# Eden-Kramer-Lab/spectral_connectivity

Measured on AMD Instinct MI355X. Metric: channel-pair*freq-bins/s for CSM+coherence(+wPLI), higher is better.
Workload: dtype f32

## Files before the change

spectral_connectivity_amd/csrc/sc_fused2.hip:

```cpp
#include <stdlib.h>
#include "sc_fused_common.h"

typedef _Float16 h16x4 __attribute__((ext_vector_type(4)));
typedef _Float16 h16x8 __attribute__((ext_vector_type(8)));
typedef _Float16 h16x2 __attribute__((ext_vector_type(2)));
typedef __attribute__((address_space(3))) unsigned char lds_u8;
typedef short s16x4 __attribute__((ext_vector_type(4)));
typedef __attribute__((address_space(3))) s16x4 lds_s16x4;

#define F2_GROUP 1056
#define F2_PLANE (8 * F2_GROUP + 64)
#define F2_NPL 6
#define F2_HPL 4
#define F2_BUF (F2_NPL * F2_PLANE)
#define F2_NBUF 3
#define F2_SCALE_OFF (F2_NBUF * F2_BUF)
#define F2_LDS (F2_SCALE_OFF + 512)
#define F2_ROW_TILE 256

extern "C" int64_t sc_planes_scales_work_bytes(int64_t n_rows, int64_t width);
extern "C" int64_t sc_planes_row_bytes(int64_t n_signals) { return (int64_t)F2_ROW_TILE * ((n_signals + 31) / 32); }

__device__ __forceinline__ unsigned f2_pack(float lo, float hi) {
    const h16x2 v = {(_Float16)lo, (_Float16)hi};
    return __builtin_bit_cast(unsigned, v);
}
__device__ __forceinline__ float f2_lo(unsigned p) { return (float)__builtin_bit_cast(h16x2, p)[0]; }
__device__ __forceinline__ float f2_hi(unsigned p) { return (float)__builtin_bit_cast(h16x2, p)[1]; }
__device__ __forceinline__ void f2_split2(float x0, float x1, unsigned& h, unsigned& m) {
    h = f2_pack(x0, x1);
    m = f2_pack(x0 - f2_lo(h), x1 - f2_hi(h));
}

__device__ __forceinline__ float planes_mag(float v) {
    const float a = fabsf(v);
    return a <= 3.4028234e38f ? a : 0.f;
}
__device__ __forceinline__ float planes_fin(float v) { return fabsf(v) <= 3.4028234e38f ? v : 0.f; }
__global__ void __launch_bounds__(256) planes_absmax_kernel(const float* x, int64_t n_rows, int width, int comps, unsigned* mx, float* part) {
    __shared__ unsigned red[2048];
    __shared__ float sred[2048];
    const int64_t rows_per_block = (n_rows + gridDim.x - 1) / gridDim.x;
    const int64_t r0 = (int64_t)blockIdx.x * rows_per_block, r1 = r0 + rows_per_block < n_rows ? r0 + rows_per_block : n_rows;
    const int tid = threadIdx.x;
    auto ord = [](float v) -> unsigned { const unsigned u = __float_as_uint(v); return (u & 0x80000000u) ? ~u : (u | 0x80000000u); };
    if ((width & 3) == 0 && width <= 1024 && (((uintptr_t)x) & 15) == 0 && r0 < r1) {
        const int q = width >> 2;
        const int rows_per_step = 256 / q;
        const int cq = tid % q, ro = tid / q;
        for (int i = tid; i < 2 * width; i += 256) red[i] = 0u;
        __syncthreads();
        if (ro < rows_per_step) {
            float4 pv = make_float4(0.f, 0.f, 0.f, 0.f);
            if (part) {
                pv = *reinterpret_cast<const float4*>(x + r0 * width + 4 * cq);
                pv.x = planes_fin(pv.x); pv.y = planes_fin(pv.y); pv.z = planes_fin(pv.z); pv.w = planes_fin(pv.w);
            }
            float4 hi = make_float4(-3.4e38f, -3.4e38f, -3.4e38f, -3.4e38f), lo = hi;
            float4 m = make_float4(0.f, 0.f, 0.f, 0.f), s1 = m, s2 = m;
            auto take = [&](const float4 v) {
                if (part) {
                    const float a0 = planes_fin(v.x), a1 = planes_fin(v.y), a2 = planes_fin(v.z), a3 = planes_fin(v.w);
                    const bool f0 = fabsf(v.x) <= 3.4028234e38f, f1 = fabsf(v.y) <= 3.4028234e38f, f2 = fabsf(v.z) <= 3.4028234e38f,
                               f3 = fabsf(v.w) <= 3.4028234e38f;
                    hi.x = fmaxf(hi.x, f0 ? a0 : hi.x); hi.y = fmaxf(hi.y, f1 ? a1 : hi.y); hi.z = fmaxf(hi.z, f2 ? a2 : hi.z); hi.w = fmaxf(hi.w, f3 ? a3 : hi.w);
                    lo.x = fmaxf(lo.x, f0 ? -a0 : lo.x); lo.y = fmaxf(lo.y, f1 ? -a1 : lo.y); lo.z = fmaxf(lo.z, f2 ? -a2 : lo.z); lo.w = fmaxf(lo.w, f3 ? -a3 : lo.w);
                    const float d0 = f0 ? a0 - pv.x : 0.f, d1 = f1 ? a1 - pv.y : 0.f, d2 = f2 ? a2 - pv.z : 0.f, d3 = f3 ? a3 - pv.w : 0.f;
                    s1.x += d0; s1.y += d1; s1.z += d2; s1.w += d3;
                    s2.x = fmaf(d0, d0, s2.x); s2.y = fmaf(d1, d1, s2.y); s2.z = fmaf(d2, d2, s2.z); s2.w = fmaf(d3, d3, s2.w);
                } else {
                    m.x = fmaxf(m.x, planes_mag(v.x)); m.y = fmaxf(m.y, planes_mag(v.y));
                    m.z = fmaxf(m.z, planes_mag(v.z)); m.w = fmaxf(m.w, planes_mag(v.w));
                }
            };
            int64_t r = r0 + ro;
            for (; r + 3 * rows_per_step < r1; r += 4 * rows_per_step) {
                float4 v[4];
#pragma unroll
                for (int u = 0; u < 4; ++u) v[u] = *reinterpret_cast<const float4*>(x + (r + (int64_t)u * rows_per_step) * width + 4 * cq);
#pragma unroll
                for (int u = 0; u < 4; ++u) take(v[u]);
            }
            for (; r < r1; r += rows_per_step) take(*reinterpret_cast<const float4*>(x + r * width + 4 * cq));
            if (part) {
                atomicMax(red + 4 * cq, ord(hi.x)); atomicMax(red + 4 * cq + 1, ord(hi.y)); atomicMax(red + 4 * cq + 2, ord(hi.z)); atomicMax(red + 4 * cq + 3, ord(hi.w));
                atomicMax(red + width + 4 * cq, ord(lo.x)); atomicMax(red + width + 4 * cq + 1, ord(lo.y));
                atomicMax(red + width + 4 * cq + 2, ord(lo.z)); atomicMax(red + width + 4 * cq + 3, ord(lo.w));
                float* sr = sred + (ro * width + 4 * cq) * 2;
                sr[0] = s1.x; sr[1] = s2.x; sr[2] = s1.y; sr[3] = s2.y; sr[4] = s1.z; sr[5] = s2.z; sr[6] = s1.w; sr[7] = s2.w;
            } else {
                atomicMax(red + 4 * cq, __float_as_uint(m.x)); atomicMax(red + 4 * cq + 1, __float_as_uint(m.y));
                atomicMax(red + 4 * cq + 2, __float_as_uint(m.z)); atomicMax(red + 4 * cq + 3, __float_as_uint(m.w));
            }
        }
        __syncthreads();
        for (int col = tid; col < width; col += 256) {
            if (!part) {
                if (red[col]) atomicMax(mx + col / comps, red[col]);
                continue;
            }
            if (red[col]) atomicMax(mx + col, red[col]);
            if (red[width + col]) atomicMax(mx + width + col, red[width + col]);
            float t1 = 0.f, t2 = 0.f;
            for (int k = 0; k < rows_per_step; ++k) { t1 += sred[(k * width + col) * 2]; t2 += sred[(k * width + col) * 2 + 1]; }
            float* o = part + ((int64_t)blockIdx.x * width + col) * 3;
            o[0] = planes_fin(x[r0 * width + col]); o[1] = t1; o[2] = t2;
        }
        return;
    }
    for (int col = tid; col < width; col += 256) {
        float m = 0.f, hi = -3.4e38f, lo = -3.4e38f, t1 = 0.f, t2 = 0.f;
        const float pv = (part && r0 < r1) ? planes_fin(x[r0 * width + col]) : 0.f;
        bool any = false;
        for (int64_t r = r0; r < r1; ++r) {
            const float v = x[r * width + col];
            m = fmaxf(m, planes_mag(v));
            if (fabsf(v) <= 3.4028234e38f) { any = true; hi = fmaxf(hi, v); lo = fmaxf(lo, -v); const float d = v - pv; t1 += d; t2 = fmaf(d, d, t2); }
        }
        if (!part) { if (m > 0.f) atomicMax(mx + col / comps, __float_as_uint(m)); continue; }
        if (any) { atomicMax(mx + col, ord(hi)); atomicMax(mx + width + col, ord(lo)); }
        float* o = part + ((int64_t)blockIdx.x * width + col) * 3;
        o[0] = pv; o[1] = t1; o[2] = t2;
    }
}
__global__ void planes_scale_kernel(const unsigned* mx, int C, float factor, float* scale) {
    const int c = blockIdx.x * blockDim.x + threadIdx.x;
    if (c >= C) return;
    const float b = __uint_as_float(mx[c]) * factor;
    float s = 1.f;
    if (b > 0.f && b < 3.0e38f) {
        int e;
        (void)frexpf(b, &e);
        int k = 15 - e;
        k = k < -100 ? -100 : (k > 100 ? 100 : k);
        s = ldexpf(1.f, k);
    }
    scale[c] = s;
    scale[C + c] = 1.f / s;
}
__global__ void __launch_bounds__(64) planes_scale_quality_kernel(unsigned* mx, int C, float taper_abs_sum, int detrend, float* scale,
                                                                  const float* part, int n_blocks, int64_t rows_per_block, int64_t n_rows) {
    const int c = blockIdx.x, lane = threadIdx.x;
    auto unord = [](unsigned p) -> float { return __uint_as_float((p & 0x80000000u) ? (p & 0x7fffffffu) : ~p); };
    const unsigned ph = mx[c], pl = mx[C + c];
    const bool any = ph != 0u && pl != 0u;
    const float hi = any ? unord(ph) : 0.f, lo = any ? -unord(pl) : 0.f;
    const float amp = detrend ? 4.f * (hi - lo) : fmaxf(fabsf(hi), fabsf(lo));
    const float b = amp * taper_abs_sum;
    float s = 1.f;
    if (b > 0.f && b < 3.0e38f) {
        int e;
        (void)frexpf(b, &e);
        int k = 15 - e;
        k = k < -100 ? -100 : (k > 100 ? 100 : k);
        s = ldexpf(1.f, k);
    }
    if (lane == 0) { scale[c] = s; scale[C + c] = 1.f / s; }
    float quiet = 3.4e38f;
    for (int blk = lane; blk < n_blocks; blk += 64) {
        const int64_t rb = (int64_t)blk * rows_per_block;
        const double nb = (double)((rb + rows_per_block < n_rows ? rb + rows_per_block : n_rows) - rb);
        if (nb < 2.0) continue;
        const float* o = part + ((int64_t)blk * C + c) * 3;
        const double s1 = (double)o[1], s2 = (double)o[2];
        const double var = (s2 - s1 * s1 / nb) / nb, mean = (double)o[0] + s1 / nb;
        if (!(var > 1e-12 * (mean * mean + 1e-300))) continue;
        const float typ = (float)sqrt(detrend ? var : var + mean * mean);
        quiet = fminf(quiet, typ);
    }
    for (int off = 32; off >= 1; off >>= 1) quiet = fminf(quiet, __shfl_down(quiet, off, 64));
    if (lane == 0 && quiet < 3.0e38f && b > 0.f && b < 3.0e38f) atomicMin(mx + 2 * C, __float_as_uint(quiet * s));
}
static int64_t planes_stat_blocks(int64_t n_rows) {
    int64_t blocks = n_rows / 128;
    return blocks < 1 ? 1 : (blocks > 2048 ? 2048 : blocks);
}
extern "C" int64_t sc_planes_scales_work_bytes(int64_t n_rows, int64_t width) {
    return 4 * ((2 * width + 1 + 3) / 4 * 4) + 4 * 3 * planes_stat_blocks(n_rows) * width;
}
static int planes_scales(const float* d_x, int64_t n_rows, int C, int comps, float factor, float* d_scale, void* d_work, void* stream) {
    hipStream_t s = (hipStream_t)stream;
    unsigned* mx = (unsigned*)d_work;
    SC_CHECK_HIP(hipMemsetAsync(mx, 0, sizeof(unsigned) * C, s));
    hipLaunchKernelGGL(planes_absmax_kernel, dim3((unsigned)planes_stat_blocks(n_rows)), dim3(256), 0, s, d_x, n_rows, C * comps, comps, mx, (float*)nullptr);
    hipLaunchKernelGGL(planes_scale_kernel, dim3((C + 63) / 64), dim3(64), 0, s, mx, C, factor, d_scale);
    SC_CHECK_HIP(hipGetLastError());
    return SC_OK;
}
extern "C" int sc_planes_scales_from_series_f32(const float* d_x, int64_t T, int64_t R, int64_t C, double taper_abs_sum,
                                                float* d_scale, void* d_work, void* stream) {
    ScTimed timed_("planes_scales", stream);
    SC_REQUIRE(d_x && d_scale && d_work && T >= 1 && R >= 1 && C >= 1 && taper_abs_sum > 0.0, "bad argument");
    return planes_scales(d_x, T * R, (int)C, 1, (float)(8.0 * taper_abs_sum), d_scale, d_work, stream);
}
extern "C" int sc_planes_scales_quality_f32(const float* d_x, int64_t T, int64_t R, int64_t C, int detrend_type, double taper_abs_sum,
                                            float* d_scale, void* d_work, int64_t work_bytes, float* d_quality, void* stream) {
    ScTimed timed_("planes_scales", stream);
    SC_REQUIRE(d_x && d_scale && d_work && d_quality && T >= 1 && R >= 1 && C >= 1 && taper_abs_sum > 0.0, "bad argument");
    SC_REQUIRE(detrend_type >= 0 && detrend_type <= 2, "unknown detrend_type");
    SC_REQUIRE(work_bytes >= sc_planes_scales_work_bytes(T * R, C), "work buffer smaller than sc_planes_scales_work_bytes");
    hipStream_t s = (hipStream_t)stream;
    unsigned* mx = (unsigned*)d_work;
    const int64_t n_rows = T * R, blocks = planes_stat_blocks(n_rows), head = (2 * C + 1 + 3) / 4 * 4;
    float* part = (float*)d_work + head;
    SC_CHECK_HIP(hipMemsetAsync(mx, 0, sizeof(unsigned) * 2 * C, s));
    SC_CHECK_HIP(hipMemsetAsync(mx + 2 * C, 0x7f, sizeof(unsigned), s));
    hipLaunchKernelGGL(planes_absmax_kernel, dim3((unsigned)blocks), dim3(256), 0, s, d_x, n_rows, (int)C, 1, mx, part);
    hipLaunchKernelGGL(planes_scale_quality_kernel, dim3((unsigned)C), dim3(64), 0, s, mx, (int)C, (float)taper_abs_sum,
                       detrend_type != SC_DETREND_NONE ? 1 : 0, d_scale, part, (int)blocks, (n_rows + blocks - 1) / blocks, n_rows);
    SC_CHECK_HIP(hipMemcpyAsync(d_quality, mx + 2 * C, sizeof(float), hipMemcpyDeviceToDevice, s));
    SC_CHECK_HIP(hipGetLastError());
    return SC_OK;
}
extern "C" int sc_planes_scales_from_spectra_f32(const void* d_X, int64_t n_rows, int64_t C, float* d_scale, void* d_work, void* stream) {
    SC_REQUIRE(d_X && d_scale && d_work && n_rows >= 1 && C >= 1, "bad argument");
    return planes_scales((const float*)d_X, n_rows, (int)C, 2, 1.0f, d_scale, d_work, stream);
}

struct PlanesConvArgs {
    const float2* X;
    unsigned char* P;
    const float* scale;
    int64_t sF, sW, sR, sK;
    int F, W, R, K, C, nct;
    int64_t n_rows;
};
__global__ void __launch_bounds__(256) planes_from_spectra_kernel(PlanesConvArgs a) {
    const int pairs_per_row = a.nct * 16;
    const int64_t i = (int64_t)blockIdx.x * 256 + threadIdx.x;
    if (i >= a.n_rows * pairs_per_row) return;
    const int64_t row = i / pairs_per_row;
    const int pr = (int)(i - row * pairs_per_row), c = 2 * pr;
    int64_t t = row;
    const int k = (int)(t % a.K); t /= a.K;
    const int r = (int)(t % a.R); t /= a.R;
    const int w = (int)(t % a.W); t /= a.W;
    const int f = (int)t;
    const float2* src = a.X + (int64_t)f * a.sF + (int64_t)w * a.sW + (int64_t)r * a.sR + (int64_t)k * a.sK + c;
    float2 v0 = make_float2(0.f, 0.f), v1 = v0;
    if (c < a.C) { const float s0 = a.scale[c]; v0 = src[0]; v0.x *= s0; v0.y *= s0; }
    if (c + 1 < a.C) { const float s1 = a.scale[c + 1]; v1 = src[1]; v1.x *= s1; v1.y *= s1; }
    unsigned* dst = reinterpret_cast<unsigned*>(a.P + row * (int64_t)a.nct * F2_ROW_TILE + (pr >> 4) * F2_ROW_TILE) + (pr & 15);
    unsigned rh, rm, ih, im;
    f2_split2(v0.x, v1.x, rh, rm);
    f2_split2(v0.y, v1.y, ih, im);
    dst[0] = rh; dst[16] = rm; dst[32] = ih; dst[48] = im;
}
__global__ void __launch_bounds__(256) spectra_from_planes_kernel(PlanesConvArgs a) {
    const int pairs_per_row = a.nct * 16;
    const int64_t i = (int64_t)blockIdx.x * 256 + threadIdx.x;
    if (i >= a.n_rows * pairs_per_row) return;
    const int64_t row = i / pairs_per_row;
    const int pr = (int)(i - row * pairs_per_row), c = 2 * pr;
    if (c >= a.C) return;
    int64_t t = row;
    const int k = (int)(t % a.K); t /= a.K;
    const int r = (int)(t % a.R); t /= a.R;
    const int w = (int)(t % a.W); t /= a.W;
    const int f = (int)t;
    const unsigned* src = reinterpret_cast<const unsigned*>(a.P + row * (int64_t)a.nct * F2_ROW_TILE + (pr >> 4) * F2_ROW_TILE) + (pr & 15);
    const unsigned rh = src[0], rm = src[16], ih = src[32], im = src[48];
    const float i0 = a.scale[a.C + c], i1 = (c + 1 < a.C) ? a.scale[a.C + c + 1] : 1.f;
    const float2 v0 = make_float2((f2_lo(rh) + f2_lo(rm)) * i0, (f2_lo(ih) + f2_lo(im)) * i0);
    const float2 v1 = make_float2((f2_hi(rh) + f2_hi(rm)) * i1, (f2_hi(ih) + f2_hi(im)) * i1);
    float2* dst = const_cast<float2*>(a.X) + (int64_t)f * a.sF + (int64_t)w * a.sW + (int64_t)r * a.sR + (int64_t)k * a.sK + c;
    dst[0] = v0;
    if (c + 1 < a.C) dst[1] = v1;
}
static int planes_conv(const void* d_X, const sc_spectra_desc* d, const float* d_scale, void* d_P, bool to_planes, void* stream) {
    SC_REQUIRE(d_X && d && d_P && d_scale, "NULL argument");
    SC_REQUIRE(d->n_freq >= 1 && d->n_windows >= 1 && d->n_trials >= 1 && d->n_tapers >= 1 && d->n_signals >= 1, "empty dimension");
    PlanesConvArgs a;
    a.X = (const float2*)d_X; a.P = (unsigned char*)d_P; a.scale = d_scale;
    a.sF = d->stride_freq; a.sW = d->stride_window; a.sR = d->stride_trial; a.sK = d->stride_taper;
    a.F = (int)d->n_freq; a.W = (int)d->n_windows; a.R = (int)d->n_trials; a.K = (int)d->n_tapers; a.C = (int)d->n_signals;
    a.nct = (a.C + 31) / 32;
    a.n_rows = (int64_t)a.F * a.W * a.R * a.K;
    const int64_t items = a.n_rows * a.nct * 16;
    const unsigned blocks = (unsigned)((items + 255) / 256);
    if (to_planes) hipLaunchKernelGGL(planes_from_spectra_kernel, dim3(blocks), dim3(256), 0, (hipStream_t)stream, a);
    else hipLaunchKernelGGL(spectra_from_planes_kernel, dim3(blocks), dim3(256), 0, (hipStream_t)stream, a);
    SC_CHECK_HIP(hipGetLastError());
    return SC_OK;
}
extern "C" int sc_planes_from_spectra_f32(const void* d_X, const sc_spectra_desc* desc, const float* d_scale, void* d_P, void* stream) {
    ScTimed timed_("planes_from_spectra", stream);
    return planes_conv(d_X, desc, d_scale, d_P, true, stream);
}
extern "C" int sc_spectra_from_planes_f32(const void* d_P, const sc_spectra_desc* desc, const float* d_scale, void* d_X, void* stream) {
    ScTimed timed_("spectra_from_planes", stream);
    return planes_conv(d_X, desc, d_scale, const_cast<void*>(d_P), false, stream);
}

struct Fused2Args {
    FusedArgs f;
    const unsigned char* P;
    const float* inv_scale;
    int64_t row_bytes;
    int64_t obs_rows;
    int loader_csm;
    int terms4;
    int fold_obs;
};

__device__ __forceinline__ h16x4 f2_tr(lds_u8* base, int off) {
    return __builtin_bit_cast(h16x4, __builtin_amdgcn_ds_read_tr16_b64_v4i16((lds_s16x4*)(base + off)));
}
__device__ __forceinline__ h16x8 f2_frag(lds_u8* base, int p) {
    const h16x4 a = f2_tr(base, p * F2_PLANE), b = f2_tr(base, p * F2_PLANE + 256);
    const h16x8 v = {a[0], a[1], a[2], a[3], b[0], b[1], b[2], b[3]};
    return v;
}

#define F2_MFMA(a, b, c) c = __builtin_amdgcn_mfma_f32_16x16x32_f16(a, b, c, 0, 0, 0)

struct F2Loader {
    const unsigned char* src;
    unsigned voff;
    int lds_off;
    int o7_0, plane;
    int n_inst;
};
template <int NHALF>
__device__ __forceinline__ F2Loader f2_loader(const Fused2Args& a, int wave, const unsigned char* part_base) {
    F2Loader L;
    const int lane = fu_lane();
    const int piece = lane & 15, ct = NHALF == 2 ? ((piece >> 2) & 1) : (piece >> 2), half = NHALF == 2 ? (piece >> 3) : 0;
    if (a.loader_csm) {
        L.plane = wave < 4 ? wave : -1;
        L.o7_0 = 0;
        L.n_inst = 8;
    } else {
        L.plane = wave >= 4 ? ((wave - 4) & 3) : -1;
        L.o7_0 = wave >= 4 ? 4 * ((wave - 4) >> 2) : 0;
        L.n_inst = 4;
    }
    L.voff = (unsigned)((8 * (lane >> 4) + FU_OC * half) * a.obs_rows * a.row_bytes + fu_byte(a.f.map.off32, ct) * F2_ROW_TILE + (piece & 3) * 16);
    L.src = part_base + (L.plane < 0 ? 0 : L.plane) * 64;
    L.lds_off = (L.plane < 0 ? 0 : L.plane) * F2_PLANE + L.o7_0 * F2_GROUP;
    return L;
}
template <int NHALF>
__device__ __forceinline__ void f2_issue(const Fused2Args& a, const F2Loader& L, lds_u8* buf, int o0, int n_left) {
    if (L.plane < 0) return;
    const int lane = fu_lane();
    const int ct = NHALF == 2 ? ((lane >> 2) & 1) : ((lane & 15) >> 2);
    const bool lane_ok = ct < a.f.NB32 && fu_byte(a.f.map.n32, ct) > 0;
    const int o_first = L.o7_0 + 8 * (lane >> 4) + (NHALF == 2 ? FU_OC * ((lane >> 3) & 1) : 0);
#pragma unroll
    for (int i = 0; i < 8; ++i) {
        if (i >= L.n_inst) break;
        lds_u8* dst = buf + L.lds_off + i * F2_GROUP;
        const unsigned char* src = L.src + (int64_t)(o0 + L.o7_0 + i) * a.obs_rows * a.row_bytes;
        if (lane_ok && o_first + i < n_left)
            asm volatile("s_mov_b32 m0, %0\n\ts_nop 0\n\tglobal_load_lds_dwordx4 %1, %2"
                         :: "s"((unsigned)reinterpret_cast<uintptr_t>(dst)), "v"(L.voff), "s"(src) : "memory", "m0");
    }
}
template <int NHALF>
__device__ __forceinline__ void f2_finish(const F2Loader& L, lds_u8* buf, int n_left) {
    if (L.plane < 0) return;
    const int lane = fu_lane();
    if (n_left < FU_OC * NHALF) {
#pragma unroll
        for (int i = 0; i < 8; ++i) {
            if (i >= L.n_inst) break;
            const int o = L.o7_0 + i + 8 * (lane >> 4) + (NHALF == 2 ? FU_OC * ((lane >> 3) & 1) : 0);
            if (o >= n_left)
                *reinterpret_cast<__attribute__((address_space(3))) u32x4*>(buf + L.lds_off + i * F2_GROUP + 16 * lane) = (u32x4){0u, 0u, 0u, 0u};
        }
    }
    if (L.plane < 2) {
#pragma unroll
        for (int i = 0; i < 8; ++i) {
            if (i >= L.n_inst) break;
            lds_u8* g = buf + L.lds_off + i * F2_GROUP + 16 * lane;
            u32x4 v = *reinterpret_cast<__attribute__((address_space(3))) u32x4*>(g);
            v[0] ^= 0x80008000u; v[1] ^= 0x80008000u; v[2] ^= 0x80008000u; v[3] ^= 0x80008000u;
            *reinterpret_cast<__attribute__((address_space(3))) u32x4*>(g + 4 * F2_PLANE) = v;
        }
    }
}

__device__ __forceinline__ int f2_issued(const F2Loader& L, int n_left) {
    if (L.plane < 0) return 0;
    const int k = n_left - L.o7_0;
    return k < 0 ? 0 : (k > L.n_inst ? L.n_inst : k);
}
__device__ __forceinline__ void f2_wait_loads(int outstanding) {
    switch (outstanding) {
    case 8: asm volatile("s_waitcnt vmcnt(8)" ::: "memory"); break;
    case 7: asm volatile("s_waitcnt vmcnt(7)" ::: "memory"); break;
    case 6: asm volatile("s_waitcnt vmcnt(6)" ::: "memory"); break;
    case 5: asm volatile("s_waitcnt vmcnt(5)" ::: "memory"); break;
    case 4: asm volatile("s_waitcnt vmcnt(4)" ::: "memory"); break;
    case 3: asm volatile("s_waitcnt vmcnt(3)" ::: "memory"); break;
    case 2: asm volatile("s_waitcnt vmcnt(2)" ::: "memory"); break;
    case 1: asm volatile("s_waitcnt vmcnt(1)" ::: "memory"); break;
    default: asm volatile("s_waitcnt vmcnt(0)" ::: "memory"); break;
    }
}

template <int NB32>
__device__ __forceinline__ void f2_mfma_role(const Fused2Args& a, lds_u8* lds, const unsigned char* lds_generic, const F2Loader& L,
                                             int wave, float* rec, int n_part) {
    const FusedArgs& p = a.f;
    constexpr int MAXS = 2 * NB32 + 1;
    constexpr int NHALF = NB32 <= 2 ? 2 : 1, CH = FU_OC * NHALF;
    const int FLUSH = a.fold_obs / CH;
    const unsigned sg = (unsigned)__builtin_amdgcn_readfirstlane((int)(wave == 0 ? p.seg0 : (wave == 1 ? p.seg1 : (wave == 2 ? p.seg2 : p.seg3))));
    const unsigned sg_n = (unsigned)__builtin_amdgcn_readfirstlane((int)((p.seg_n >> (8 * wave)) & 0xffu));
    const int rA_ = sg & 0xf, cA_ = (sg >> 4) & 0xf, rB_ = (sg >> 8) & 0xf, cB_ = (sg >> 12) & 0xf;
    const int nA_ = sg_n & 0xf, nB_ = sg_n >> 4;
    const int total = nA_ + nB_;
    f32x4 re[MAXS], im[MAXS];
#pragma unroll
    for (int s = 0; s < MAXS; ++s) { re[s] = (f32x4){0.f, 0.f, 0.f, 0.f}; im[s] = re[s]; }
    const int n_chunks = (n_part + CH - 1) / CH;
    float* out = rec + (int64_t)p.csm_plane * p.n_tiles * SC_TILE_ELEMS;
    const bool do_csm = p.csm_plane >= 0 && (p.debug_skip & 1) == 0;
    const bool loads = !(p.debug_skip & 8);
    const bool t4 = a.terms4 != 0;
    for (int ch = 0; ch < n_chunks; ++ch) {
        lds_u8* cur = lds + (loads ? (ch % F2_NBUF) : 0) * F2_BUF;
        const bool more = ch + 1 < n_chunks && loads, more2 = ch + 2 < n_chunks && loads;
        if (more2) f2_issue<NHALF>(a, L, lds + ((ch + 2) % F2_NBUF) * F2_BUF, (ch + 2) * CH, n_part - (ch + 2) * CH);
        if (do_csm && total > 0) {
            int rA = rA_, rB = rB_, nA = nA_, cA = cA_, cB = cB_;
            asm volatile("" : "+s"(rA), "+s"(rB), "+s"(nA), "+s"(cA), "+s"(cB));
            const int lane = fu_lane(), g = lane >> 4;
            lds_u8* b00 = cur + ((4 * (g & 1) + ((lane >> 2) & 3)) * F2_GROUP + 2 * (g >> 1) * 256 + (lane & 3) * 8);
            h16x8 arh, arm, aih, aim, nrh, nrm;
#pragma unroll
            for (int hv = 0; hv < NHALF; ++hv) {
            lds_u8* b0 = b00 + hv * 128;
#pragma unroll
            for (int s = 0; s < MAXS; ++s) {
                if (s < total) {
                    const bool in_a = s < nA;
                    const int row = in_a ? rA : rB;
                    const int col = in_a ? cA + s : cB + (s - nA);
                    if (s == 0 || s == nA) {
                        lds_u8* fa = b0 + row * 32;
                        arh = f2_frag(fa, 0); arm = f2_frag(fa, 1); aih = f2_frag(fa, 2); aim = f2_frag(fa, 3);
                        nrh = f2_frag(fa, 4); nrm = f2_frag(fa, 5);
                    }
                    lds_u8* fb = b0 + col * 32;
                    const h16x8 brh = f2_frag(fb, 0), bih = f2_frag(fb, 2), brm = f2_frag(fb, 1), bim = f2_frag(fb, 3);
                    F2_MFMA(arh, brh, re[s]);  F2_MFMA(aih, brh, im[s]);
                    F2_MFMA(aih, bih, re[s]);  F2_MFMA(nrh, bih, im[s]);
                    F2_MFMA(arh, brm, re[s]);  F2_MFMA(aih, brm, im[s]);
                    F2_MFMA(aih, bim, re[s]);  F2_MFMA(nrh, bim, im[s]);
                    F2_MFMA(arm, brh, re[s]);  F2_MFMA(aim, brh, im[s]);
                    F2_MFMA(aim, bih, re[s]);  F2_MFMA(nrm, bih, im[s]);
                    if (t4) {
                        F2_MFMA(arm, brm, re[s]);  F2_MFMA(aim, brm, im[s]);
                        F2_MFMA(aim, bim, re[s]);  F2_MFMA(nrm, bim, im[s]);
                    }
                }
            }
            }
        }
        if (more && L.plane >= 0) {
            f2_wait_loads(more2 ? f2_issued(L, n_part - (ch + 2) * CH) : 0);
            f2_finish<NHALF>(L, lds + ((ch + 1) % F2_NBUF) * F2_BUF, n_part - (ch + 1) * CH);
        }
        {
            const bool last = ch + 1 == n_chunks;
#pragma unroll
            for (int s = 0; s < MAXS; ++s) {
                const int f_s = FLUSH - 1 - s;
                const bool due = ((ch + 1 + s) % FLUSH) == 0 && !(p.debug_skip & 64);
                if (s < total && (due || last) && p.csm_plane >= 0) {
                    const bool first = ch <= f_s || (p.debug_skip & 64);
                    const bool in_a = s < nA_;
                    const int row = in_a ? rA_ : rB_;
                    const int col = in_a ? cA_ + s : cB_ + (s - nA_);
                    float* o_re = out + (int64_t)sc_tile_index(fu_gt(p.map, row), fu_gt(p.map, col), p.map.NBr) * SC_TILE_ELEMS;
                    float* o_im = o_re + (int64_t)p.n_tiles * SC_TILE_ELEMS;
                    const unsigned fl = (unsigned)fu_lane();
                    const unsigned base_idx = (fl >> 4) * 64u + (fl & 15u);
                    const float* isc = reinterpret_cast<const float*>((const unsigned char*)lds_generic + F2_SCALE_OFF);
                    const float sj = isc[col * 16 + (int)(fl & 15u)];
                    const f32x4 si = *reinterpret_cast<const f32x4*>(isc + row * 16 + 4 * (int)(fl >> 4));
#pragma unroll
                    for (int r = 0; r < 4; ++r) {
                        const unsigned idx = base_idx + 16u * r;
                        const float sc = sj * si[r];
                        if (first) {
                            o_re[idx] = re[s][r] * sc;
                            o_im[idx] = im[s][r] * sc;
                        } else {
                            unsafeAtomicAdd(o_re + idx, re[s][r] * sc);
                            unsafeAtomicAdd(o_im + idx, im[s][r] * sc);
                        }
                    }
                    re[s] = (f32x4){0.f, 0.f, 0.f, 0.f}; im[s] = re[s];
                }
            }
        }
        F2_BARRIER();
    }
    const int wps = 8 / p.n_sets;
    for (int half = wps >> 1; half >= 1; half >>= 1) { __syncthreads(); __syncthreads(); }
}

template <int NB32, int COL_LO, int ROW_HI, int SET, int OP, int RPW>
__device__ __forceinline__ void f2_valu_body(const Fused2Args& a, lds_u8* lds, unsigned char* smem, const F2Loader& L, int tid,
                                             int rsub, int wps, float* rec, int n_part) {
    const FusedArgs& p = a.f;
    using Tab = FuTab<NB32, COL_LO, ROW_HI, SET>;
    constexpr int NBLK = Tab::NBLK;
    constexpr bool PK = NBLK <= 4 && fu_nsets(NB32, COL_LO, ROW_HI) == 1;
// ... 307 lines not shown
```

Baseline: 2.788 billion.

## Split quality scan into dedicated kernel with per-slab records, drop memsets and global atomics

Adds a dedicated planes_scan_kernel that writes per-slab records (pivot, sums, hi/lo ordered max) in a column-major layout. The merge kernel then reduces those records per channel with a wave shuffle instead of using global atomicMax. The scan is software-pipelined with a 6-deep register prefetch and sched barriers. The separate memsets and the device-to-device copy of the quality value are removed, since the quality word is initialized inside the scan kernel and written directly. The aim is to cut launch and API overhead and atomic traffic in the scale/quality stage, at the cost of a larger work buffer and more per-channel merge reads.

```diff
diff --git a/spectral_connectivity_amd/csrc/sc_fused2.hip b/spectral_connectivity_amd/csrc/sc_fused2.hip
--- a/spectral_connectivity_amd/csrc/sc_fused2.hip
+++ b/spectral_connectivity_amd/csrc/sc_fused2.hip
@@ -37,41 +37,26 @@
     return a <= 3.4028234e38f ? a : 0.f;
 }
 __device__ __forceinline__ float planes_fin(float v) { return fabsf(v) <= 3.4028234e38f ? v : 0.f; }
-__global__ void __launch_bounds__(256) planes_absmax_kernel(const float* x, int64_t n_rows, int width, int comps, unsigned* mx, float* part) {
-    __shared__ unsigned red[2048];
-    __shared__ float sred[2048];
+static int64_t planes_stat_blocks(int64_t n_rows) {
+    int64_t blocks = n_rows / 128;
+    return blocks < 1 ? 1 : (blocks > 2048 ? 2048 : blocks);
+}
+__global__ void __launch_bounds__(256) planes_absmax_kernel(const float* x, int64_t n_rows, int width, int comps, unsigned* mx) {
+    __shared__ unsigned red[1024];
     const int64_t rows_per_block = (n_rows + gridDim.x - 1) / gridDim.x;
     const int64_t r0 = (int64_t)blockIdx.x * rows_per_block, r1 = r0 + rows_per_block < n_rows ? r0 + rows_per_block : n_rows;
     const int tid = threadIdx.x;
-    auto ord = [](float v) -> unsigned { const unsigned u = __float_as_uint(v); return (u & 0x80000000u) ? ~u : (u | 0x80000000u); };
     if ((width & 3) == 0 && width <= 1024 && (((uintptr_t)x) & 15) == 0 && r0 < r1) {
         const int q = width >> 2;
         const int rows_per_step = 256 / q;
         const int cq = tid % q, ro = tid / q;
-        for (int i = tid; i < 2 * width; i += 256) red[i] = 0u;
+        for (int i = tid; i < width; i += 256) red[i] = 0u;
         __syncthreads();
         if (ro < rows_per_step) {
-            float4 pv = make_float4(0.f, 0.f, 0.f, 0.f);
-            if (part) {
-                pv = *reinterpret_cast<const float4*>(x + r0 * width + 4 * cq);
-                pv.x = planes_fin(pv.x); pv.y = planes_fin(pv.y); pv.z = planes_fin(pv.z); pv.w = planes_fin(pv.w);
-            }
-            float4 hi = make_float4(-3.4e38f, -3.4e38f, -3.4e38f, -3.4e38f), lo = hi;
-            float4 m = make_float4(0.f, 0.f, 0.f, 0.f), s1 = m, s2 = m;
+            float4 m = make_float4(0.f, 0.f, 0.f, 0.f);
             auto take = [&](const float4 v) {
-                if (part) {
-                    const float a0 = planes_fin(v.x), a1 = planes_fin(v.y), a2 = planes_fin(v.z), a3 = planes_fin(v.w);
-                    const bool f0 = fabsf(v.x) <= 3.4028234e38f, f1 = fabsf(v.y) <= 3.4028234e38f, f2 = fabsf(v.z) <= 3.4028234e38f,
-                               f3 = fabsf(v.w) <= 3.4028234e38f;
-                    hi.x = fmaxf(hi.x, f0 ? a0 : hi.x); hi.y = fmaxf(hi.y, f1 ? a1 : hi.y); hi.z = fmaxf(hi.z, f2 ? a2 : hi.z); hi.w = fmaxf(hi.w, f3 ? a3 : hi.w);
-                    lo.x = fmaxf(lo.x, f0 ? -a0 : lo.x); lo.y = fmaxf(lo.y, f1 ? -a1 : lo.y); lo.z = fmaxf(lo.z, f2 ? -a2 : lo.z); lo.w = fmaxf(lo.w, f3 ? -a3 : lo.w);
-                    const float d0 = f0 ? a0 - pv.x : 0.f, d1 = f1 ? a1 - pv.y : 0.f, d2 = f2 ? a2 - pv.z : 0.f, d3 = f3 ? a3 - pv.w : 0.f;
-                    s1.x += d0; s1.y += d1; s1.z += d2; s1.w += d3;
-                    s2.x = fmaf(d0, d0, s2.x); s2.y = fmaf(d1, d1, s2.y); s2.z = fmaf(d2, d2, s2.z); s2.w = fmaf(d3, d3, s2.w);
-                } else {
-                    m.x = fmaxf(m.x, planes_mag(v.x)); m.y = fmaxf(m.y, planes_mag(v.y));
-                    m.z = fmaxf(m.z, planes_mag(v.z)); m.w = fmaxf(m.w, planes_mag(v.w));
-                }
+                m.x = fmaxf(m.x, planes_mag(v.x)); m.y = fmaxf(m.y, planes_mag(v.y));
+                m.z = fmaxf(m.z, planes_mag(v.z)); m.w = fmaxf(m.w, planes_mag(v.w));
             };
             int64_t r = r0 + ro;
             for (; r + 3 * rows_per_step < r1; r += 4 * rows_per_step) {
@@ -82,45 +67,18 @@
                 for (int u = 0; u < 4; ++u) take(v[u]);
             }
             for (; r < r1; r += rows_per_step) take(*reinterpret_cast<const float4*>(x + r * width + 4 * cq));
-            if (part) {
-                atomicMax(red + 4 * cq, ord(hi.x)); atomicMax(red + 4 * cq + 1, ord(hi.y)); atomicMax(red + 4 * cq + 2, ord(hi.z)); atomicMax(red + 4 * cq + 3, ord(hi.w));
-                atomicMax(red + width + 4 * cq, ord(lo.x)); atomicMax(red + width + 4 * cq + 1, ord(lo.y));
-                atomicMax(red + width + 4 * cq + 2, ord(lo.z)); atomicMax(red + width + 4 * cq + 3, ord(lo.w));
-                float* sr = sred + (ro * width + 4 * cq) * 2;
-                sr[0] = s1.x; sr[1] = s2.x; sr[2] = s1.y; sr[3] = s2.y; sr[4] = s1.z; sr[5] = s2.z; sr[6] = s1.w; sr[7] = s2.w;
-            } else {
-                atomicMax(red + 4 * cq, __float_as_uint(m.x)); atomicMax(red + 4 * cq + 1, __float_as_uint(m.y));
-                atomicMax(red + 4 * cq + 2, __float_as_uint(m.z)); atomicMax(red + 4 * cq + 3, __float_as_uint(m.w));
-            }
+            atomicMax(red + 4 * cq, __float_as_uint(m.x)); atomicMax(red + 4 * cq + 1, __float_as_uint(m.y));
+            atomicMax(red + 4 * cq + 2, __float_as_uint(m.z)); atomicMax(red + 4 * cq + 3, __float_as_uint(m.w));
         }
         __syncthreads();
-        for (int col = tid; col < width; col += 256) {
-            if (!part) {
-                if (red[col]) atomicMax(mx + col / comps, red[col]);
-                continue;
-            }
-            if (red[col]) atomicMax(mx + col, red[col]);
-            if (red[width + col]) atomicMax(mx + width + col, red[width + col]);
-            float t1 = 0.f, t2 = 0.f;
-            for (int k = 0; k < rows_per_step; ++k) { t1 += sred[(k * width + col) * 2]; t2 += sred[(k * width + col) * 2 + 1]; }
-            float* o = part + ((int64_t)blockIdx.x * width + col) * 3;
-            o[0] = planes_fin(x[r0 * width + col]); o[1] = t1; o[2] = t2;
-        }
+        for (int col = tid; col < width; col += 256)
+            if (red[col]) atomicMax(mx + col / comps, red[col]);
         return;
     }
     for (int col = tid; col < width; col += 256) {
-        float m = 0.f, hi = -3.4e38f, lo = -3.4e38f, t1 = 0.f, t2 = 0.f;
-        const float pv = (part && r0 < r1) ? planes_fin(x[r0 * width + col]) : 0.f;
-        bool any = false;
-        for (int64_t r = r0; r < r1; ++r) {
-            const float v = x[r * width + col];
-            m = fmaxf(m, planes_mag(v));
-            if (fabsf(v) <= 3.4028234e38f) { any = true; hi = fmaxf(hi, v); lo = fmaxf(lo, -v); const float d = v - pv; t1 += d; t2 = fmaf(d, d, t2); }
-        }
-        if (!part) { if (m > 0.f) atomicMax(mx + col / comps, __float_as_uint(m)); continue; }
-        if (any) { atomicMax(mx + col, ord(hi)); atomicMax(mx + width + col, ord(lo)); }
-        float* o = part + ((int64_t)blockIdx.x * width + col) * 3;
-        o[0] = pv; o[1] = t1; o[2] = t2;
+        float m = 0.f;
+        for (int64_t r = r0; r < r1; ++r) m = fmaxf(m, planes_mag(x[r * width + col]));
+        if (m > 0.f) atomicMax(mx + col / comps, __float_as_uint(m));
     }
 }
 __global__ void planes_scale_kernel(const unsigned* mx, int C, float factor, float* scale) {
@@ -138,11 +96,137 @@
     scale[c] = s;
     scale[C + c] = 1.f / s;
 }
-__global__ void __launch_bounds__(64) planes_scale_quality_kernel(unsigned* mx, int C, float taper_abs_sum, int detrend, float* scale,
-                                                                  const float* part, int n_blocks, int64_t rows_per_block, int64_t n_rows) {
+#define PLANES_SCAN_ROWS 6
+#define PLANES_NO_CHANNEL 0x7f7f7f7fu
+__global__ void __launch_bounds__(256, 8) planes_scan_kernel(const float* x, int64_t n_rows, int width, unsigned* rec, unsigned* quality) {
+    __shared__ uint4 sred[1024];
+    const int n_blocks = gridDim.x, slab = blockIdx.x;
+    const int64_t rows_per_block = (n_rows + n_blocks - 1) / n_blocks;
+    const int64_t r0 = (int64_t)slab * rows_per_block, r1 = r0 + rows_per_block < n_rows ? r0 + rows_per_block : n_rows;
+    const int tid = threadIdx.x;
+    if (blockIdx.x == 0 && tid == 0) *quality = PLANES_NO_CHANNEL;
+    auto ord = [](float v) -> unsigned { const unsigned u = __float_as_uint(v); return (u & 0x80000000u) ? ~u : (u | 0x80000000u); };
+    auto put = [&](int col, float pivot, float t1, float t2, unsigned hi, unsigned lo) {
+        unsigned* o = rec + ((int64_t)col * n_blocks + slab) * 5;
+        o[0] = __float_as_uint(pivot); o[1] = __float_as_uint(t1); o[2] = __float_as_uint(t2); o[3] = hi; o[4] = lo;
+    };
+    if ((width & 3) == 0 && width <= 1024 && (((uintptr_t)x) & 15) == 0 && r0 < r1) {
+        const int q = width >> 2;
+        const int rows_per_step = 256 / q;
+        const int cq = tid % q, ro = tid / q;
+        const float* xb = x + r0 * width;
+        const float p0 = tid < width ? xb[tid] : 0.f;
+        if (ro < rows_per_step) {
+            float4 pv = *reinterpret_cast<const float4*>(xb + 4 * cq);
+            pv.x = planes_fin(pv.x); pv.y = planes_fin(pv.y); pv.z = planes_fin(pv.z); pv.w = planes_fin(pv.w);
+            float4 hi = make_float4(-3.4e38f, -3.4e38f, -3.4e38f, -3.4e38f), lo = hi;
+            float4 s1 = make_float4(0.f, 0.f, 0.f, 0.f), s2 = s1;
+            auto take = [&](const float4 v) {
+                const float a0 = planes_fin(v.x), a1 = planes_fin(v.y), a2 = planes_fin(v.z), a3 = planes_fin(v.w);
+                const bool f0 = fabsf(v.x) <= 3.4028234e38f, f1 = fabsf(v.y) <= 3.4028234e38f, f2 = fabsf(v.z) <= 3.4028234e38f,
+                           f3 = fabsf(v.w) <= 3.4028234e38f;
+                hi.x = fmaxf(hi.x, f0 ? a0 : hi.x); hi.y = fmaxf(hi.y, f1 ? a1 : hi.y); hi.z = fmaxf(hi.z, f2 ? a2 : hi.z); hi.w = fmaxf(hi.w, f3 ? a3 : hi.w);
+                lo.x = fmaxf(lo.x, f0 ? -a0 : lo.x); lo.y = fmaxf(lo.y, f1 ? -a1 : lo.y); lo.z = fmaxf(lo.z, f2 ? -a2 : lo.z); lo.w = fmaxf(lo.w, f3 ? -a3 : lo.w);
+                const float d0 = f0 ? a0 - pv.x : 0.f, d1 = f1 ? a1 - pv.y : 0.f, d2 = f2 ? a2 - pv.z : 0.f, d3 = f3 ? a3 - pv.w : 0.f;
+                s1.x += d0; s1.y += d1; s1.z += d2; s1.w += d3;
+                s2.x = fmaf(d0, d0, s2.x); s2.y = fmaf(d1, d1, s2.y); s2.z = fmaf(d2, d2, s2.z); s2.w = fmaf(d3, d3, s2.w);
+            };
+            const int slab_rows = (int)(r1 - r0), step = rows_per_step * width;
+            const int mine = (slab_rows - ro + rows_per_step - 1) / rows_per_step;
+            const int full = slab_rows / rows_per_step / PLANES_SCAN_ROWS * PLANES_SCAN_ROWS;
+            const unsigned toff = (unsigned)(ro * width + 4 * cq);
+            const float* xs = xb;
+            float4 v[PLANES_SCAN_ROWS];
+            auto load = [&](int u) { v[u] = *reinterpret_cast<const float4*>(xs + u * step + toff); };
+            auto load_end = [&](int u) { v[u] = *reinterpret_cast<const float4*>(full + u < mine ? xs + u * step + toff : xb + 4 * cq); };
+            if (full > 0) {
+#pragma unroll
+                for (int u = 0; u < PLANES_SCAN_ROWS; ++u) load(u);
+                for (int k = PLANES_SCAN_ROWS; k < full; k += PLANES_SCAN_ROWS) {
+                    xs += (int64_t)PLANES_SCAN_ROWS * step;
+#pragma unroll
+                    for (int u = 0; u < PLANES_SCAN_ROWS; ++u) { take(v[u]); load(u); __builtin_amdgcn_sched_barrier(0); }
+                }
+                xs += (int64_t)PLANES_SCAN_ROWS * step;
+#pragma unroll
+                for (int u = 0; u < PLANES_SCAN_ROWS; ++u) { take(v[u]); load_end(u); __builtin_amdgcn_sched_barrier(0); }
+            } else {
+#pragma unroll
+                for (int u = 0; u < PLANES_SCAN_ROWS; ++u) load_end(u);
+            }
+#pragma unroll
+            for (int u = 0; u < PLANES_SCAN_ROWS; ++u)
+                if (full + u < mine) take(v[u]);
+            uint4* sr = sred + ro * width + 4 * cq;
+            sr[0] = make_uint4(__float_as_uint(s1.x), __float_as_uint(s2.x), ord(hi.x), ord(lo.x));
+            sr[1] = make_uint4(__float_as_uint(s1.y), __float_as_uint(s2.y), ord(hi.y), ord(lo.y));
+            sr[2] = make_uint4(__float_as_uint(s1.z), __float_as_uint(s2.z), ord(hi.z), ord(lo.z));
+            sr[3] = make_uint4(__float_as_uint(s1.w), __float_as_uint(s2.w), ord(hi.w), ord(lo.w));
+        }
+        __syncthreads();
+#pragma unroll
+        for (int j = 0; j < 4; ++j) {
+            const int col = tid + 256 * j;
+            if (col >= width) break;
+            float t1 = 0.f, t2 = 0.f;
+            unsigned ph = 0u, pl = 0u;
+            for (int k = 0; k < rows_per_step; ++k) {
+                const uint4 e = sred[k * width + col];
+                t1 += __uint_as_float(e.x); t2 += __uint_as_float(e.y);
+                ph = e.z > ph ? e.z : ph; pl = e.w > pl ? e.w : pl;
+            }
+            put(col, planes_fin(j == 0 ? p0 : xb[col]), t1, t2, ph, pl);
+        }
+        return;
+    }
+    for (int col = tid; col < width; col += 256) {
+        float hi = -3.4e38f, lo = -3.4e38f, t1 = 0.f, t2 = 0.f;
+        const float pv = r0 < r1 ? planes_fin(x[r0 * width + col]) : 0.f;
+        bool any = false;
+        for (int64_t r = r0; r < r1; ++r) {
+            const float v = x[r * width + col];
+            if (fabsf(v) <= 3.4028234e38f) { any = true; hi = fmaxf(hi, v); lo = fmaxf(lo, -v); const float d = v - pv; t1 += d; t2 = fmaf(d, d, t2); }
+        }
+        put(col, pv, t1, t2, any ? ord(hi) : 0u, any ? ord(lo) : 0u);
+    }
+}
+#define PLANES_MERGE_RECS 4
+__global__ void __launch_bounds__(64) planes_scale_quality_kernel(const unsigned* rec, int C, float taper_abs_sum, int detrend, float* scale,
+                                                                  unsigned* quality, int n_blocks, int64_t rows_per_block, int64_t n_rows) {
     const int c = blockIdx.x, lane = threadIdx.x;
+    const unsigned* rc = rec + (int64_t)c * n_blocks * 5;
     auto unord = [](unsigned p) -> float { return __uint_as_float((p & 0x80000000u) ? (p & 0x7fffffffu) : ~p); };
-    const unsigned ph = mx[c], pl = mx[C + c];
+    unsigned ph = 0u, pl = 0u;
+    float quiet = 3.4e38f;
+    for (int b0 = lane; b0 < n_blocks; b0 += 64 * PLANES_MERGE_RECS) {
+        unsigned w[PLANES_MERGE_RECS][5];
+#pragma unroll
+        for (int u = 0; u < PLANES_MERGE_RECS; ++u) {
+            const int blk = b0 + 64 * u;
+            const unsigned* o = rc + (int64_t)(blk < n_blocks ? blk : b0) * 5;
+#pragma unroll
+            for (int i = 0; i < 5; ++i) w[u][i] = o[i];
+        }
+#pragma unroll
+        for (int u = 0; u < PLANES_MERGE_RECS; ++u) {
+            const int blk = b0 + 64 * u;
+            if (blk >= n_blocks) continue;
+            ph = w[u][3] > ph ? w[u][3] : ph;
+            pl = w[u][4] > pl ? w[u][4] : pl;
+            const int64_t rb = (int64_t)blk * rows_per_block;
+            const double nb = (double)((rb + rows_per_block < n_rows ? rb + rows_per_block : n_rows) - rb);
+            if (nb < 2.0) continue;
+            const double s1 = (double)__uint_as_float(w[u][1]), s2 = (double)__uint_as_float(w[u][2]);
+            const double var = (s2 - s1 * s1 / nb) / nb, mean = (double)__uint_as_float(w[u][0]) + s1 / nb;
+            if (!(var > 1e-12 * (mean * mean + 1e-300))) continue;
+            const float typ = (float)sqrt(detrend ? var : var + mean * mean);
+            quiet = fminf(quiet, typ);
+        }
+    }
+    for (int off = 32; off >= 1; off >>= 1) {
+        const unsigned oh = __shfl_xor(ph, off, 64), ol = __shfl_xor(pl, off, 64);
+        ph = oh > ph ? oh : ph; pl = ol > pl ? ol : pl;
+    }
     const bool any = ph != 0u && pl != 0u;
     const float hi = any ? unord(ph) : 0.f, lo = any ? -unord(pl) : 0.f;
     const float amp = detrend ? 4.f * (hi - lo) : fmaxf(fabsf(hi), fabsf(lo));
@@ -156,33 +240,17 @@
         s = ldexpf(1.f, k);
     }
     if (lane == 0) { scale[c] = s; scale[C + c] = 1.f / s; }
-    float quiet = 3.4e38f;
-    for (int blk = lane; blk < n_blocks; blk += 64) {
-        const int64_t rb = (int64_t)blk * rows_per_block;
-        const double nb = (double)((rb + rows_per_block < n_rows ? rb + rows_per_block : n_rows) - rb);
-        if (nb < 2.0) continue;
-        const float* o = part + ((int64_t)blk * C + c) * 3;
-        const double s1 = (double)o[1], s2 = (double)o[2];
-        const double var = (s2 - s1 * s1 / nb) / nb, mean = (double)o[0] + s1 / nb;
-        if (!(var > 1e-12 * (mean * mean + 1e-300))) continue;
-        const float typ = (float)sqrt(detrend ? var : var + mean * mean);
-        quiet = fminf(quiet, typ);
-    }
     for (int off = 32; off >= 1; off >>= 1) quiet = fminf(quiet, __shfl_down(quiet, off, 64));
-    if (lane == 0 && quiet < 3.0e38f && b > 0.f && b < 3.0e38f) atomicMin(mx + 2 * C, __float_as_uint(quiet * s));
-}
-static int64_t planes_stat_blocks(int64_t n_rows) {
-    int64_t blocks = n_rows / 128;
-    return blocks < 1 ? 1 : (blocks > 2048 ? 2048 : blocks);
+    if (lane == 0 && quiet < 3.0e38f && b > 0.f && b < 3.0e38f) atomicMin(quality, __float_as_uint(quiet * s));
 }
 extern "C" int64_t sc_planes_scales_work_bytes(int64_t n_rows, int64_t width) {
-    return 4 * ((2 * width + 1 + 3) / 4 * 4) + 4 * 3 * planes_stat_blocks(n_rows) * width;
+    return 4 * 5 * planes_stat_blocks(n_rows) * width;
 }
 static int planes_scales(const float* d_x, int64_t n_rows, int C, int comps, float factor, float* d_scale, void* d_work, void* stream) {
     hipStream_t s = (hipStream_t)stream;
     unsigned* mx = (unsigned*)d_work;
     SC_CHECK_HIP(hipMemsetAsync(mx, 0, sizeof(unsigned) * C, s));
-    hipLaunchKernelGGL(planes_absmax_kernel, dim3((unsigned)planes_stat_blocks(n_rows)), dim3(256), 0, s, d_x, n_rows, C * comps, comps, mx, (float*)nullptr);
+    hipLaunchKernelGGL(planes_absmax_kernel, dim3((unsigned)planes_stat_blocks(n_rows)), dim3(256), 0, s, d_x, n_rows, C * comps, comps, mx);
     hipLaunchKernelGGL(planes_scale_kernel, dim3((C + 63) / 64), dim3(64), 0, s, mx, C, factor, d_scale);
     SC_CHECK_HIP(hipGetLastError());
     return SC_OK;
@@ -200,15 +268,11 @@
     SC_REQUIRE(detrend_type >= 0 && detrend_type <= 2, "unknown detrend_type");
     SC_REQUIRE(work_bytes >= sc_planes_scales_work_bytes(T * R, C), "work buffer smaller than sc_planes_scales_work_bytes");
     hipStream_t s = (hipStream_t)stream;
-    unsigned* mx = (unsigned*)d_work;
-    const int64_t n_rows = T * R, blocks = planes_stat_blocks(n_rows), head = (2 * C + 1 + 3) / 4 * 4;
-    float* part = (float*)d_work + head;
-    SC_CHECK_HIP(hipMemsetAsync(mx, 0, sizeof(unsigned) * 2 * C, s));
-    SC_CHECK_HIP(hipMemsetAsync(mx + 2 * C, 0x7f, sizeof(unsigned), s));
-    hipLaunchKernelGGL(planes_absmax_kernel, dim3((unsigned)blocks), dim3(256), 0, s, d_x, n_rows, (int)C, 1, mx, part);
-    hipLaunchKernelGGL(planes_scale_quality_kernel, dim3((unsigned)C), dim3(64), 0, s, mx, (int)C, (float)taper_abs_sum,
-                       detrend_type != SC_DETREND_NONE ? 1 : 0, d_scale, part, (int)blocks, (n_rows + blocks - 1) / blocks, n_rows);
-    SC_CHECK_HIP(hipMemcpyAsync(d_quality, mx + 2 * C, sizeof(float), hipMemcpyDeviceToDevice, s));
+    unsigned* rec = (unsigned*)d_work;
+    const int64_t n_rows = T * R, blocks = planes_stat_blocks(n_rows);
+    hipLaunchKernelGGL(planes_scan_kernel, dim3((unsigned)blocks), dim3(256), 0, s, d_x, n_rows, (int)C, rec, (unsigned*)d_quality);
+    hipLaunchKernelGGL(planes_scale_quality_kernel, dim3((unsigned)C), dim3(64), 0, s, rec, (int)C, (float)taper_abs_sum,
+                       detrend_type != SC_DETREND_NONE ? 1 : 0, d_scale, (unsigned*)d_quality, (int)blocks, (n_rows + blocks - 1) / blocks, n_rows);
     SC_CHECK_HIP(hipGetLastError());
     return SC_OK;
 }
```

After: 2.786 billion (median of 2 runs). Within noise of the previous version (-0.1%).
